# das-ankur/Efficient-PIC-with-Variance-Aware-Masking

Hardware: AMD Instinct MI355X
Metric: megapixels/sec encode+decode (g_a->mask->g_s) at 256x256 bs32 (higher is better)
Workload: dtype f32 (bf16x3 split operands); 1 GPU; forward_single_quality q=2.5 on 32x3x256x256 per GPU (dual g_a, hyperprior, 10 base + 10 progressive slices, variance mask, likelihood, LRP, g_s[1]); README model N=192 M=640; batch_per_gpu=32, global_batch=32, hip_graph=True, weights=synthetic seed 0

## Files before the change

efficient-pic-with-variance-aware-masking_amd/csrc/conv_igemm.hip:

```cpp
#include "common.h"
#include <cstdlib>

namespace vam {

typedef float f32x16 __attribute__((ext_vector_type(16)));
typedef unsigned int u32x4 __attribute__((ext_vector_type(4)));
typedef __bf16 bf16x8 __attribute__((ext_vector_type(8)));
typedef _Float16 f16x8 __attribute__((ext_vector_type(8)));
typedef _Float16 f16x2 __attribute__((ext_vector_type(2)));

struct ConvP {
  const float* seg_ptr[VAM_MAX_SEG];
  int seg_ld[VAM_MAX_SEG];
  int seg_end[VAM_MAX_SEG];
  int n_seg;
  int H, W, HW;
  int kh, kw, stride, pad_y, pad_x;
  int Ho, Wo, HoWo;
  int P;
  int N, Npad;
  int Cin, Kc, Kc16;
  const float* wpack;
  const float* bias;
  float* out;
  int ldo, Hf, Wf, osy, osx, ooy, oox, Cq, act, flags;
  const float* pre;
  const float* mul;
  const float* post;
  const float* post2;
  int ld_pre, ld_mul, ld_post, ld_post2;
  float* preact;
  int ld_preact;
  int tiles_n;
  const int* in_amax[VAM_MAX_SEG];
  int* out_amax;
};

constexpr int VAM_CONVI_DUAL = 1 << 29;
constexpr int VAM_CONVI_STAGED = 1 << 30;

struct GroupArgs {
  int nprob;
  int staged_epilogue;
  int tile_start[VAM_MAX_GROUP + 1];
  ConvP p[VAM_MAX_GROUP];
};

__device__ __forceinline__ float apply_act(float v, int act) {
  switch (act) {
    case VAM_ACT_GELU: return vam_gelu(v);
    case VAM_ACT_LEAKY: return v > 0.f ? v : v * 0.01f;
    case VAM_ACT_HALF_TANH: return 0.5f * tanhf(v);
    case VAM_ACT_SIGMOID: return 1.0f / (1.0f + expf(-v));
    case VAM_ACT_CLAMP01: return fminf(fmaxf(v, 0.f), 1.f);
    case VAM_ACT_RSQRT: return 1.0f / sqrtf(v);
    case VAM_ACT_SQRT: return sqrtf(v);
    case VAM_ACT_DOUBLE: return 2.0f * v;
    default: return v;
  }
}

constexpr int PK = 16;

template <int BM, int BN, int BK, int WGM, int WGN, int MODE, int AIN = 0, int SPEC = 0>
__global__ __launch_bounds__(WGM * WGN * 64 * (SPEC ? 2 : 1), SPEC ? ((BM + BN <= 192) ? 4 : 2) : (((MODE == 1 || MODE == 3) && BM == 128 && BN == 128) ? 3 : 2)) void conv_igemm_kernel(const GroupArgs args) {
  static_assert(SPEC == 0 || MODE == 1 || MODE == 3, "wave specialisation is built for the split-operand modes");
  static_assert(MODE != 3 || AIN == 0, "MODE 3 (fp16x2) takes fp32 inputs");
  static_assert(MODE != 2 || AIN <= 1, "MODE 2: AIN 0 = fp32 input rounded while staged, 1 = bf16 input");
  constexpr int NT = WGM * WGN * 64;
  constexpr int NTC = NT;
  constexpr int NTB = NT * (SPEC ? 2 : 1);
  constexpr int LDS_LD = BK;
  constexpr int TM = BM / WGM / 32;
  constexpr int TN = BN / WGN / 32;
  constexpr int CPR = MODE ? 4 : BK / 4;
  constexpr int LDW = MODE ? 8 : 4;
  static_assert(MODE == 0 || BK == 32, "the bf16 paths step K by 32 channels");
  constexpr int SW_SHIFT = (CPR == 4) ? 2 : 1;
  constexpr int RPP = NT / CPR;
  constexpr int NA = (BM + RPP - 1) / RPP;
  constexpr int NB = (BN + RPP - 1) / RPP;
  constexpr bool A_FULL = (BM % RPP) == 0, B_FULL = (BN % RPP) == 0;
  static_assert(TM >= 1 && TN >= 1 && BM == TM * WGM * 32 && BN == TN * WGN * 32, "tile/wave layout");

  extern __shared__ __attribute__((aligned(16))) float smem[];
  float* sA = smem;
  float* sB = smem + 2 * BM * LDS_LD;

  int pi = -1, t = 0;
  {
    const int xcd = blockIdx.x & 7;
    int idx = blockIdx.x >> 3;
#pragma unroll
    for (int i = 0; i < VAM_MAX_GROUP; ++i) {
      if (i < args.nprob && pi < 0) {
        const int T = args.tile_start[i + 1] - args.tile_start[i];
        const int q = T >> 3, r = T & 7;
        const int c = q + (xcd < r ? 1 : 0);
        if (idx < c) {
          pi = i;
          t = xcd * q + (xcd < r ? xcd : r) + idx;
        } else {
          idx -= c;
        }
      }
    }
  }
  if (pi < 0) return;
  const ConvP& P = args.p[pi];
  const int u_kh = __builtin_amdgcn_readfirstlane(P.kh), u_kw = __builtin_amdgcn_readfirstlane(P.kw);
  const int u_W = __builtin_amdgcn_readfirstlane(P.W), u_Kc = __builtin_amdgcn_readfirstlane(P.Kc);
  const int u_kc16 = __builtin_amdgcn_readfirstlane(P.Kc16), u_Npad = __builtin_amdgcn_readfirstlane(P.Npad);
  const int u_se0 = __builtin_amdgcn_readfirstlane(P.seg_end[0]), u_se1 = __builtin_amdgcn_readfirstlane(P.seg_end[1]);
  const int u_se2 = __builtin_amdgcn_readfirstlane(P.seg_end[2]);
  const int tn = t % P.tiles_n, tm = t / P.tiles_n;
  const int m0 = tm * BM, n0 = tn * BN;

  const bool is_loader = SPEC && (__builtin_amdgcn_readfirstlane((int)threadIdx.x >> 6) >= WGM * WGN);
  const int tid = (SPEC && (int)threadIdx.x >= NTC) ? (int)threadIdx.x - NTC : (int)threadIdx.x;
  const int lane = tid & 63, wid = tid >> 6;
  const int wm = wid / WGN, wn = wid % WGN;
  const int ld_row = tid / CPR;
  const int ld_col = (tid % CPR) * LDW;

  int a_pix0[NA];
  unsigned a_mask[NA];
#pragma unroll
  for (int i = 0; i < NA; ++i) {
    int p = m0 + ld_row + i * RPP;
    a_pix0[i] = 0;
    a_mask[i] = 0u;
    if (p < P.P && (A_FULL || ld_row + i * RPP < BM)) {
      int b = p / P.HoWo;
      int r = p - b * P.HoWo;
      int oy = r / P.Wo;
      int ox = r - oy * P.Wo;
      const int iy0 = oy * P.stride - P.pad_y, ix0 = ox * P.stride - P.pad_x;
      a_pix0[i] = b * P.HW + iy0 * P.W + ix0;
      unsigned m = 0u;
      for (int ty = 0; ty < u_kh; ++ty)
        for (int tx = 0; tx < u_kw; ++tx)
          if ((unsigned)(iy0 + ty) < (unsigned)P.H && (unsigned)(ix0 + tx) < (unsigned)P.W) m |= 1u << (ty * u_kw + tx);
      a_mask[i] = m;
    }
  }
  f32x16 acc[TM][TN];
  if constexpr (!SPEC) {
#pragma unroll
    for (int i = 0; i < TM; ++i)
#pragma unroll
      for (int j = 0; j < TN; ++j)
#pragma unroll
        for (int r = 0; r < 16; ++r) acc[i][j][r] = 0.f;
  }

  const int l31 = lane & 31, lh = lane >> 5;
  const unsigned long long wpa = reinterpret_cast<unsigned long long>(P.wpack);
  const __amdgpu_buffer_rsrc_t rsrc_w = __builtin_amdgcn_make_buffer_rsrc(
      reinterpret_cast<void*>(((unsigned long long)(unsigned)__builtin_amdgcn_readfirstlane((unsigned)(wpa >> 32)) << 32) |
                              (unsigned long long)(unsigned)__builtin_amdgcn_readfirstlane((unsigned)wpa)), 0, 0x7FFFFFFF, 0x00020000);
  const bool sq = (P.flags & VAM_CONV_SQUARE_IN) != 0;

  int c_ty = 0, c_tx = 0, c_kc = 0, c_tap = 0;
  int s_begin = 0, s_end = 0, s_ld4 = 0;
  unsigned s_lo = 0, s_hi = 0;
  const int n_taps = u_kh * u_kw;
  const bool dual = (MODE == 1 || MODE == 3) && (P.flags & VAM_CONVI_DUAL) != 0;
  const int n_chunks = dual ? (n_taps + 1) / 2 : n_taps * u_Kc;
  constexpr bool DIRECT_CFG = !SPEC && BM == 128 && BN == 64;
  const bool direct_out = DIRECT_CFG && !args.staged_epilogue &&
                          (P.flags & (VAM_CONV_OUT_NCHW | VAM_CONV_OUT_BF3 | VAM_CONV_OUT_BF16 | VAM_CONV_AUX_BF16 | VAM_CONVI_STAGED)) == 0;
  const int kc16 = u_kc16;
  if constexpr (MODE == 0) {
    unsigned b_off[NB];
  #pragma unroll
    for (int i = 0; i < NB; ++i) {
      const int r = ld_row + i * RPP;
      const bool ok = (B_FULL || r < BN) && (n0 + r < P.Npad);
      b_off[i] = ok ? (unsigned)((((ld_col >> 4) * u_Npad + n0 + r) * PK + (ld_col & 15)) * 4) : 0x80000000u;
    }
    float4 ra0[NA], rb0[NB], ra1[NA], rb1[NB];


    auto gload = [&](float4 (&ra)[NA], float4 (&rb)[NB]) {
      const int cc0 = c_kc * BK;
      if (cc0 < s_begin || cc0 >= s_end) {
        const int k = (cc0 >= u_se0 ? 1 : 0) + (cc0 >= u_se1 ? 1 : 0) + (cc0 >= u_se2 ? 1 : 0);
        s_begin = __builtin_amdgcn_readfirstlane(k ? P.seg_end[k - 1] : 0);
        s_end = __builtin_amdgcn_readfirstlane(P.seg_end[k]);
        const unsigned long long spa = reinterpret_cast<unsigned long long>(P.seg_ptr[k]);
        s_lo = (unsigned)__builtin_amdgcn_readfirstlane((unsigned)spa);
        s_hi = (unsigned)__builtin_amdgcn_readfirstlane((unsigned)(spa >> 32));
        s_ld4 = __builtin_amdgcn_readfirstlane(P.seg_ld[k]) * 4;
      }
      const int seg_begin = s_begin;
      const int sld4 = s_ld4;
      const __amdgpu_buffer_rsrc_t rsrc_a = __builtin_amdgcn_make_buffer_rsrc(
          reinterpret_cast<void*>(((unsigned long long)s_hi << 32) | s_lo), 0, 0x7FFFFFFF, 0x00020000);
      const int tap_pix = c_ty * u_W + c_tx;
      const int col4 = (cc0 - seg_begin + ld_col) * 4;
  #pragma unroll
      for (int i = 0; i < NA; ++i) {
        const bool ok = (a_mask[i] >> c_tap) & 1u;
        const unsigned off = (unsigned)((a_pix0[i] + tap_pix) * sld4 + col4);
        const u32x4 v = __builtin_amdgcn_raw_buffer_load_b128(rsrc_a, (int)(ok ? off : 0x80000000u), 0, 0);
        float4 f = make_float4(__uint_as_float(v.x), __uint_as_float(v.y), __uint_as_float(v.z), __uint_as_float(v.w));
        ra[i] = sq ? make_float4(f.x * f.x, f.y * f.y, f.z * f.z, f.w * f.w) : f;
      }
      const unsigned wbase = (unsigned)((c_tap * kc16 + c_kc * (BK / PK)) * u_Npad * (PK * 4));
  #pragma unroll
      for (int i = 0; i < NB; ++i) {
        const u32x4 v = __builtin_amdgcn_raw_buffer_load_b128(rsrc_w, (int)(b_off[i] + wbase), 0, 0);
        rb[i] = make_float4(__uint_as_float(v.x), __uint_as_float(v.y), __uint_as_float(v.z), __uint_as_float(v.w));
      }
      if (BK == 16) {
        const int has_half = (((c_kc & 1) == 0) && (c_kc + 1 < kc16)) ? 1 : 0;
        const int adv_tap = has_half ? 0 : 1;
        c_kc += has_half;
        c_tap += adv_tap;
        c_tx += adv_tap;
        const int wx = (c_tx == u_kw) ? 1 : 0;
        c_tx = wx ? 0 : c_tx;
        c_ty += wx;
        const int wt = (c_tap == n_taps) ? 1 : 0;
        c_tap = wt ? 0 : c_tap;
        c_ty = wt ? 0 : c_ty;
        c_kc = adv_tap ? (wt ? (c_kc | 1) + 1 : (c_kc & ~1)) : c_kc;
      } else {
        ++c_tap;
        ++c_tx;
        const int wx = (c_tx == u_kw) ? 1 : 0;
        c_tx = wx ? 0 : c_tx;
        c_ty += wx;
        const int wt = (c_tap == n_taps) ? 1 : 0;
        c_tap = wt ? 0 : c_tap;
        c_ty = wt ? 0 : c_ty;
        c_kc += wt;
      }
    };
    static_assert(RPP % 16 == 0, "the swizzle of a thread's rows must not depend on the pass");
    const int st_col = (((ld_col >> 2) ^ ((ld_row >> SW_SHIFT) & (CPR - 1))) << 2);
    auto sstore = [&](int buf, const float4 (&ra)[NA], const float4 (&rb)[NB]) {
      float* a = sA + buf * BM * LDS_LD;
      float* b = sB + buf * BN * LDS_LD;
  #pragma unroll
      for (int i = 0; i < NA; ++i)
        if (A_FULL || ld_row + i * RPP < BM)
          *reinterpret_cast<float4*>(a + (ld_row + i * RPP) * LDS_LD + st_col) = ra[i];
  #pragma unroll
      for (int i = 0; i < NB; ++i)
        if (B_FULL || ld_row + i * RPP < BN)
          *reinterpret_cast<float4*>(b + (ld_row + i * RPP) * LDS_LD + st_col) = rb[i];
    };

    const int a_row0 = (wm * TM * 32 + l31) * LDS_LD;
    const int b_row0 = (wn * TN * 32 + l31) * LDS_LD;
    const int rd_sw = (l31 >> SW_SHIFT) & (CPR - 1);
    int rd_col[BK / 8];
  #pragma unroll
    for (int kk = 0; kk < BK / 8; ++kk) rd_col[kk] = ((kk * 2 + lh) ^ rd_sw) << 2;

    auto compute = [&](int buf) {
      const float* a = sA + buf * BM * LDS_LD + a_row0;
      const float* b = sB + buf * BN * LDS_LD + b_row0;
      float4 fa[2][TM], fb[2][TN];
  #pragma unroll
      for (int i = 0; i < TM; ++i) fa[0][i] = *reinterpret_cast<const float4*>(a + i * 32 * LDS_LD + rd_col[0]);
  #pragma unroll
      for (int j = 0; j < TN; ++j) fb[0][j] = *reinterpret_cast<const float4*>(b + j * 32 * LDS_LD + rd_col[0]);
  #pragma unroll
      for (int kk = 0; kk < BK / 8; ++kk) {
        const int cur = kk & 1, nxt = cur ^ 1;
        if (kk + 1 < BK / 8) {
  #pragma unroll
          for (int i = 0; i < TM; ++i) fa[nxt][i] = *reinterpret_cast<const float4*>(a + i * 32 * LDS_LD + rd_col[kk + 1]);
  #pragma unroll
          for (int j = 0; j < TN; ++j) fb[nxt][j] = *reinterpret_cast<const float4*>(b + j * 32 * LDS_LD + rd_col[kk + 1]);
        }
  #pragma unroll
        for (int i = 0; i < TM; ++i)
  #pragma unroll
          for (int j = 0; j < TN; ++j) {
            acc[i][j] = __builtin_amdgcn_mfma_f32_32x32x2f32(fa[cur][i].x, fb[cur][j].x, acc[i][j], 0, 0, 0);
            acc[i][j] = __builtin_amdgcn_mfma_f32_32x32x2f32(fa[cur][i].y, fb[cur][j].y, acc[i][j], 0, 0, 0);
            acc[i][j] = __builtin_amdgcn_mfma_f32_32x32x2f32(fa[cur][i].z, fb[cur][j].z, acc[i][j], 0, 0, 0);
            acc[i][j] = __builtin_amdgcn_mfma_f32_32x32x2f32(fa[cur][i].w, fb[cur][j].w, acc[i][j], 0, 0, 0);
          }
      }
    };

    gload(ra0, rb0);
    sstore(0, ra0, rb0);
    if (n_chunks > 1) gload(ra0, rb0);
    __syncthreads();
    int ch = 0;
    for (; ch + 3 < n_chunks; ch += 2) {
      sstore(1, ra0, rb0);
      gload(ra1, rb1);
      compute(0);
      __syncthreads();
      sstore(0, ra1, rb1);
      gload(ra0, rb0);
      compute(1);
      __syncthreads();
    }
    for (; ch < n_chunks; ch += 2) {
      if (ch + 1 < n_chunks) sstore(1, ra0, rb0);
      if (ch + 2 < n_chunks) gload(ra1, rb1);
      compute(0);
      __syncthreads();
      if (ch + 1 >= n_chunks) break;
      if (ch + 2 < n_chunks) sstore(0, ra1, rb1);
      if (ch + 3 < n_chunks) gload(ra0, rb0);
      compute(1);
      __syncthreads();
    }

  } else if constexpr (MODE == 1 || MODE == 3) {
    constexpr bool F16 = MODE == 3;
    constexpr int NPL = F16 ? 2 : 3;
    constexpr int UPR = NPL * 4;
    constexpr int RS = NPL * 16;
    constexpr int NBUF = SPEC ? 2 : ((BM + BN <= 128) ? 2 : 1);
    constexpr int NBC = (BN * UPR + NT - 1) / NT;
    float* sA1 = smem;
    float* sB1 = smem + NBUF * BM * RS;
    unsigned b_goff[NBC];
    int b_loff[NBC];
#pragma unroll
    for (int j = 0; j < NBC; ++j) {
      const int idx = tid + j * NT;
      const int row = idx / UPR, c = idx - row * UPR;
      const bool in_tile = idx < BN * UPR;
      b_goff[j] = (in_tile && n0 + row < u_Npad) ? (unsigned)((n0 + row) * (UPR * 16) + c * 16) : 0x80000000u;
      b_loff[j] = in_tile ? row * RS + (F16 ? (c ^ ((row >> 1) & 7)) : ((c & ~3) | ((c & 3) ^ ((row >> 2) & 3)))) * 4 : -1;
    }
    const int u_Cin = __builtin_amdgcn_readfirstlane(P.Cin);
    float a_scale = 1.f, a_unscale = 1.f;
    if constexpr (F16) {
      int mb = 0;
#pragma unroll
      for (int k = 0; k < VAM_MAX_SEG; ++k)
        if (P.in_amax[k]) mb = max(mb, *P.in_amax[k]);
      float m = __uint_as_float((unsigned)__builtin_amdgcn_readfirstlane(mb));
      if (sq) m = m * m;
      const int e = (int)((__float_as_uint(m) >> 23) & 0xFFu) - 127;
      int sh = (m > 0.f && e > -127 && e < 128) ? 14 - e : 0;
      sh = sh > 126 ? 126 : (sh < -126 ? -126 : sh);
      a_scale = __uint_as_float((unsigned)(sh + 127) << 23);
      a_unscale = __uint_as_float((unsigned)(127 - sh) << 23);
    }
    constexpr int NAR = AIN ? 3 : 2;
    u32x4 ra0[NA][NAR], ra1[NA][NAR];
    u32x4 rb0[NBC], rb1[NBC];

    auto gload = [&](u32x4 (&ra)[NA][NAR], u32x4 (&rb)[NBC]) {
      const int cc0 = c_kc * 32;
      if (cc0 < s_begin || cc0 >= s_end) {
        const int k = (cc0 >= u_se0 ? 1 : 0) + (cc0 >= u_se1 ? 1 : 0) + (cc0 >= u_se2 ? 1 : 0);
        s_begin = __builtin_amdgcn_readfirstlane(k ? P.seg_end[k - 1] : 0);
        s_end = __builtin_amdgcn_readfirstlane(P.seg_end[k]);
        const unsigned long long spa = reinterpret_cast<unsigned long long>(P.seg_ptr[k]);
        s_lo = (unsigned)__builtin_amdgcn_readfirstlane((unsigned)spa);
        s_hi = (unsigned)__builtin_amdgcn_readfirstlane((unsigned)(spa >> 32));
        s_ld4 = __builtin_amdgcn_readfirstlane(P.seg_ld[k]) * (AIN ? 48 : 4);
      }
      const __amdgpu_buffer_rsrc_t rsrc_a = __builtin_amdgcn_make_buffer_rsrc(
          reinterpret_cast<void*>(((unsigned long long)s_hi << 32) | s_lo), 0, 0x7FFFFFFF, 0x00020000);
      int tap_pix = c_ty * u_W + c_tx;
      int col4 = AIN ? ((cc0 - s_begin + ld_col) >> 3) * 48 : (cc0 - s_begin + ld_col) * 4;
      bool ch_ok = cc0 + ld_col < u_Cin;
      int my_tap = c_tap;
      if (!AIN && dual) {
        const bool second = ld_col >= 16;
        const int txb = (c_tx + 1 == u_kw) ? 0 : c_tx + 1, tyb = (c_tx + 1 == u_kw) ? c_ty + 1 : c_ty;
        tap_pix = second ? tyb * u_W + txb : tap_pix;
        my_tap = second ? c_tap + 1 : c_tap;
        col4 = (ld_col & 15) * 4;
        ch_ok = my_tap < n_taps;
      }
#pragma unroll
      for (int i = 0; i < NA; ++i) {
        const bool ok = ch_ok && ((a_mask[i] >> my_tap) & 1u);
        const unsigned off = ok ? (unsigned)((a_pix0[i] + tap_pix) * s_ld4 + col4) : 0x80000000u;
#pragma unroll
        for (int q = 0; q < NAR; ++q) ra[i][q] = __builtin_amdgcn_raw_buffer_load_b128(rsrc_a, (int)(off + 16u * q), 0, 0);
      }
      const unsigned wbase = (unsigned)((dual ? (c_tap >> 1) : (c_tap * u_Kc + c_kc)) * u_Npad) * (unsigned)(UPR * 16);
#pragma unroll
      for (int j = 0; j < NBC; ++j) rb[j] = __builtin_amdgcn_raw_buffer_load_b128(rsrc_w, (int)(b_goff[j] + wbase), 0, 0);
      for (int step = 0; step < (dual ? 2 : 1); ++step) {
        ++c_tap;
        ++c_tx;
        const int wx = (c_tx == u_kw) ? 1 : 0;
        c_tx = wx ? 0 : c_tx;
        c_ty += wx;
      }
      const int wt = (c_tap >= n_taps) ? 1 : 0;
      c_tap = wt ? 0 : c_tap;
      c_ty = wt ? 0 : c_ty;
      c_tx = wt ? 0 : c_tx;
      c_kc += wt;
    };
    static_assert(RPP % 16 == 0, "the swizzle of a thread's rows must not depend on the pass");
    const int st1_col = (((ld_col >> 3) ^ ((ld_row >> 2) & 3)) << 2);
    const int st3_col[2] = {((((ld_col >> 3)) ^ ((ld_row >> 1) & 7)) << 2), (((4 + (ld_col >> 3)) ^ ((ld_row >> 1) & 7)) << 2)};
    auto sstore = [&](int buf, const u32x4 (&ra)[NA][NAR], const u32x4 (&rb)[NBC]) {
      float* a = sA1 + buf * BM * RS;
      float* b = sB1 + buf * BN * RS;
#pragma unroll
      for (int i = 0; i < NA; ++i)
        if (A_FULL || ld_row + i * RPP < BM) {
          if constexpr (AIN) {
            float* dst = a + (ld_row + i * RPP) * RS + st1_col;
            *reinterpret_cast<u32x4*>(dst) = ra[i][0];
            *reinterpret_cast<u32x4*>(dst + 16) = ra[i][1];
            *reinterpret_cast<u32x4*>(dst + 32) = ra[i][NAR - 1];
            continue;
          }
          float x[8] = {__uint_as_float(ra[i][0].x), __uint_as_float(ra[i][0].y), __uint_as_float(ra[i][0].z), __uint_as_float(ra[i][0].w),
                        __uint_as_float(ra[i][1].x), __uint_as_float(ra[i][1].y), __uint_as_float(ra[i][1].z), __uint_as_float(ra[i][1].w)};
          if (sq) {
#pragma unroll
            for (int e = 0; e < 8; ++e) x[e] = x[e] * x[e];
          }
          if constexpr (F16) {
            unsigned hw2[4], lw2[4];
#pragma unroll
            for (int q = 0; q < 4; ++q) {
              const float x0 = x[2 * q] * a_scale, x1 = x[2 * q + 1] * a_scale;
              const f16x2 h = {(_Float16)x0, (_Float16)x1};
              const f16x2 l = {(_Float16)(x0 - (float)h[0]), (_Float16)(x1 - (float)h[1])};
              hw2[q] = __builtin_bit_cast(unsigned, h);
              lw2[q] = __builtin_bit_cast(unsigned, l);
            }
            float* drow = a + (ld_row + i * RPP) * RS;
            u32x4 t;
            t.x = hw2[0]; t.y = hw2[1]; t.z = hw2[2]; t.w = hw2[3];
            *reinterpret_cast<u32x4*>(drow + st3_col[0]) = t;
            t.x = lw2[0]; t.y = lw2[1]; t.z = lw2[2]; t.w = lw2[3];
            *reinterpret_cast<u32x4*>(drow + st3_col[1]) = t;
            continue;
          }
          unsigned hb[8], mb[8], lb[8];
#pragma unroll
          for (int e = 0; e < 8; ++e) {
            hb[e] = __float_as_uint(x[e]);
            const float r1 = x[e] - __uint_as_float(hb[e] & 0xFFFF0000u);
            mb[e] = __float_as_uint(r1);
            lb[e] = __float_as_uint(r1 - __uint_as_float(mb[e] & 0xFFFF0000u));
          }
          unsigned hw[4], mw[4], lw[4];
#pragma unroll
          for (int q = 0; q < 4; ++q) {
            hw[q] = __builtin_amdgcn_perm(hb[2 * q + 1], hb[2 * q], 0x07060302u);
            mw[q] = __builtin_amdgcn_perm(mb[2 * q + 1], mb[2 * q], 0x07060302u);
            lw[q] = __builtin_amdgcn_perm(lb[2 * q + 1], lb[2 * q], 0x07060302u);
          }
          float* dst = a + (ld_row + i * RPP) * RS + st1_col;
          u32x4 t;
          t.x = hw[0]; t.y = hw[1]; t.z = hw[2]; t.w = hw[3];
          *reinterpret_cast<u32x4*>(dst) = t;
          t.x = mw[0]; t.y = mw[1]; t.z = mw[2]; t.w = mw[3];
          *reinterpret_cast<u32x4*>(dst + 16) = t;
          t.x = lw[0]; t.y = lw[1]; t.z = lw[2]; t.w = lw[3];
          *reinterpret_cast<u32x4*>(dst + 32) = t;
        }
#pragma unroll
      for (int j = 0; j < NBC; ++j) {
        if (b_loff[j] >= 0) *reinterpret_cast<u32x4*>(b + b_loff[j]) = rb[j];
      }
    };
    const int a_row1 = (wm * TM * 32 + l31) * RS;
    const int b_row1 = (wn * TN * 32 + l31) * RS;
    const int rsw = (l31 >> 2) & 3;
    const int rd1[2] = {((lh ^ rsw) << 2), (((2 + lh) ^ rsw) << 2)};
    const int rsw3 = (l31 >> 1) & 7;
    const int rd3[2][2] = {{((lh ^ rsw3) << 2), (((4 + lh) ^ rsw3) << 2)}, {(((2 + lh) ^ rsw3) << 2), (((6 + lh) ^ rsw3) << 2)}};
    auto compute = [&](int buf) {
      const float* a = sA1 + buf * BM * RS + a_row1;
      const float* b = sB1 + buf * BN * RS + b_row1;
      if constexpr (F16) {
#pragma unroll
        for (int ks = 0; ks < 2; ++ks) {
          f16x8 fa[TM][2], fb[TN][2];
#pragma unroll
          for (int i = 0; i < TM; ++i)
#pragma unroll
            for (int pl = 0; pl < 2; ++pl) fa[i][pl] = *reinterpret_cast<const f16x8*>(a + i * 32 * RS + rd3[ks][pl]);
#pragma unroll
          for (int j = 0; j < TN; ++j)
#pragma unroll
            for (int pl = 0; pl < 2; ++pl) fb[j][pl] = *reinterpret_cast<const f16x8*>(b + j * 32 * RS + rd3[ks][pl]);
#pragma unroll
          for (int i = 0; i < TM; ++i)
#pragma unroll
            for (int j = 0; j < TN; ++j) {
              acc[i][j] = __builtin_amdgcn_mfma_f32_32x32x16_f16(fa[i][0], fb[j][1], acc[i][j], 0, 0, 0);
              acc[i][j] = __builtin_amdgcn_mfma_f32_32x32x16_f16(fa[i][1], fb[j][0], acc[i][j], 0, 0, 0);
              acc[i][j] = __builtin_amdgcn_mfma_f32_32x32x16_f16(fa[i][0], fb[j][0], acc[i][j], 0, 0, 0);
            }
        }
        return;
      }
#pragma unroll
      for (int ks = 0; ks < 2; ++ks) {
        bf16x8 fa[TM][3], fb[TN][3];
#pragma unroll
        for (int i = 0; i < TM; ++i)
#pragma unroll
          for (int pl = 0; pl < 3; ++pl) fa[i][pl] = *reinterpret_cast<const bf16x8*>(a + i * 32 * RS + pl * 16 + rd1[ks]);
#pragma unroll
        for (int j = 0; j < TN; ++j)
#pragma unroll
          for (int pl = 0; pl < 3; ++pl) fb[j][pl] = *reinterpret_cast<const bf16x8*>(b + j * 32 * RS + pl * 16 + rd1[ks]);
#pragma unroll
        for (int i = 0; i < TM; ++i)
#pragma unroll
          for (int j = 0; j < TN; ++j) {
            acc[i][j] = __builtin_amdgcn_mfma_f32_32x32x16_bf16(fa[i][0], fb[j][2], acc[i][j], 0, 0, 0);
            acc[i][j] = __builtin_amdgcn_mfma_f32_32x32x16_bf16(fa[i][2], fb[j][0], acc[i][j], 0, 0, 0);
            acc[i][j] = __builtin_amdgcn_mfma_f32_32x32x16_bf16(fa[i][1], fb[j][1], acc[i][j], 0, 0, 0);
            acc[i][j] = __builtin_amdgcn_mfma_f32_32x32x16_bf16(fa[i][0], fb[j][1], acc[i][j], 0, 0, 0);
            acc[i][j] = __builtin_amdgcn_mfma_f32_32x32x16_bf16(fa[i][1], fb[j][0], acc[i][j], 0, 0, 0);
            acc[i][j] = __builtin_amdgcn_mfma_f32_32x32x16_bf16(fa[i][0], fb[j][0], acc[i][j], 0, 0, 0);
          }
        if constexpr (TN >= 7) __builtin_amdgcn_sched_barrier(0);
      }
    };
    auto unscale = [&]() {
      if constexpr (F16) {
        const float* wsc = P.wpack + (size_t)n_taps * u_Kc * u_Npad * 32;
#pragma unroll
        for (int j = 0; j < TN; ++j) {
          const int n = n0 + (wn * TN + j) * 32 + l31;
          const float f = (n < u_Npad ? wsc[n] : 0.f) * a_unscale;
#pragma unroll
          for (int i = 0; i < TM; ++i)
#pragma unroll
            for (int r = 0; r < 16; ++r) acc[i][j][r] *= f;
        }
      }
    };
    if constexpr (SPEC) {
      if (is_loader) {
        gload(ra0, rb0);
        if (n_chunks > 1) gload(ra1, rb1);
        sstore(0, ra0, rb0);
        if (n_chunks > 2) gload(ra0, rb0);
        __syncthreads();
        for (int ch = 0; ch < n_chunks; ch += 2) {
          if (ch + 1 < n_chunks) sstore(1, ra1, rb1);
          if (ch + 3 < n_chunks) gload(ra1, rb1);
          __syncthreads();
          if (ch + 1 >= n_chunks) break;
          if (ch + 2 < n_chunks) sstore(0, ra0, rb0);
          if (ch + 4 < n_chunks) gload(ra0, rb0);
          __syncthreads();
        }
      } else {
#pragma unroll
        for (int i = 0; i < TM; ++i)
#pragma unroll
          for (int j = 0; j < TN; ++j)
#pragma unroll
            for (int r = 0; r < 16; ++r) acc[i][j][r] = 0.f;
        __syncthreads();
        for (int ch = 0; ch < n_chunks; ch += 2) {
          compute(0);
          __syncthreads();
          if (ch + 1 >= n_chunks) break;
          compute(1);
          __syncthreads();
        }
        unscale();
        if (!direct_out) {
          float* sCf = smem;
#pragma unroll
          for (int i = 0; i < TM; ++i)
#pragma unroll
            for (int j = 0; j < TN; ++j)
#pragma unroll
              for (int r = 0; r < 16; ++r) {
                const int row = wm * TM * 32 + i * 32 + (r & 3) + 8 * (r >> 2) + 4 * lh;
                sCf[row * (BN + 4) + wn * TN * 32 + j * 32 + l31] = acc[i][j][r];
              }
        }
      }
    } else if constexpr (NBUF == 2) {
      gload(ra0, rb0);
      sstore(0, ra0, rb0);
      if (n_chunks > 1) gload(ra1, rb1);
      if (n_chunks > 2) gload(ra0, rb0);
      __syncthreads();
      int ch = 0;
      for (; ch + 1 < n_chunks; ch += 2) {
        sstore(1, ra1, rb1);
        if (ch + 3 < n_chunks) gload(ra1, rb1);
        compute(0);
        __syncthreads();
        if (ch + 2 < n_chunks) sstore(0, ra0, rb0);
        if (ch + 4 < n_chunks) gload(ra0, rb0);
        compute(1);
        __syncthreads();
      }
      if (ch < n_chunks) {
        compute(0);
        __syncthreads();
      }
      unscale();
    } else {
      gload(ra0, rb0);
      for (int ch = 0; ch < n_chunks; ++ch) {
        sstore(0, ra0, rb0);
        __syncthreads();
        if (ch + 1 < n_chunks) gload(ra0, rb0);
        compute(0);
        __syncthreads();
      }
      unscale();
    }
  } else {
    constexpr int RS = 16;
    constexpr int NBC = (BN * 4 + NT - 1) / NT;
    float* sA2 = smem;
    float* sB2 = smem + 2 * BM * RS;
    unsigned b_goff[NBC];
    int b_loff[NBC];
#pragma unroll
    for (int j = 0; j < NBC; ++j) {
      const int idx = tid + j * NT;
      const int row = idx >> 2, c = idx & 3;
      const bool in_tile = idx < BN * 4;
      b_goff[j] = (in_tile && n0 + row < u_Npad) ? (unsigned)((n0 + row) * 64 + c * 16) : 0x80000000u;
      b_loff[j] = in_tile ? row * RS + ((c ^ ((row >> 2) & 3)) << 2) : -1;
    }
    const int u_Cin = __builtin_amdgcn_readfirstlane(P.Cin);
    constexpr int NAR = AIN ? 1 : 2;
    u32x4 ra0[NA][NAR], ra1[NA][NAR];
    u32x4 rb0[NBC], rb1[NBC];
    auto gload = [&](u32x4 (&ra)[NA][NAR], u32x4 (&rb)[NBC]) {
      const int cc0 = c_kc * 32;
      if (cc0 < s_begin || cc0 >= s_end) {
        const int k = (cc0 >= u_se0 ? 1 : 0) + (cc0 >= u_se1 ? 1 : 0) + (cc0 >= u_se2 ? 1 : 0);
        s_begin = __builtin_amdgcn_readfirstlane(k ? P.seg_end[k - 1] : 0);
        s_end = __builtin_amdgcn_readfirstlane(P.seg_end[k]);
        const unsigned long long spa = reinterpret_cast<unsigned long long>(P.seg_ptr[k]);
        s_lo = (unsigned)__builtin_amdgcn_readfirstlane((unsigned)spa);
        s_hi = (unsigned)__builtin_amdgcn_readfirstlane((unsigned)(spa >> 32));
        s_ld4 = __builtin_amdgcn_readfirstlane(P.seg_ld[k]) * (AIN ? 2 : 4);
      }
      const __amdgpu_buffer_rsrc_t rsrc_a = __builtin_amdgcn_make_buffer_rsrc(
          reinterpret_cast<void*>(((unsigned long long)s_hi << 32) | s_lo), 0, 0x7FFFFFFF, 0x00020000);
      const int tap_pix = c_ty * u_W + c_tx;
      const int col4 = (cc0 - s_begin + ld_col) * (AIN ? 2 : 4);
      const bool ch_ok = cc0 + ld_col < u_Cin;
#pragma unroll
      for (int i = 0; i < NA; ++i) {
        const bool ok = ch_ok && ((a_mask[i] >> c_tap) & 1u);
        const unsigned off = ok ? (unsigned)((a_pix0[i] + tap_pix) * s_ld4 + col4) : 0x80000000u;
#pragma unroll
        for (int q = 0; q < NAR; ++q) ra[i][q] = __builtin_amdgcn_raw_buffer_load_b128(rsrc_a, (int)(off + 16u * q), 0, 0);
      }
      const unsigned wbase = (unsigned)((c_tap * u_Kc + c_kc) * u_Npad) * 64u;
#pragma unroll
      for (int j = 0; j < NBC; ++j) rb[j] = __builtin_amdgcn_raw_buffer_load_b128(rsrc_w, (int)(b_goff[j] + wbase), 0, 0);
      ++c_tap;
      ++c_tx;
      const int wx = (c_tx == u_kw) ? 1 : 0;
      c_tx = wx ? 0 : c_tx;
      c_ty += wx;
      const int wt = (c_tap == n_taps) ? 1 : 0;
      c_tap = wt ? 0 : c_tap;
      c_ty = wt ? 0 : c_ty;
      c_kc += wt;
    };
    auto pk2 = [](float lo, float hi) -> unsigned {
      const __bf16 a = (__bf16)lo, b = (__bf16)hi;
      return (unsigned)__builtin_bit_cast(unsigned short, a) | ((unsigned)__builtin_bit_cast(unsigned short, b) << 16);
    };
    const int st2_col = (((ld_col >> 3) ^ ((ld_row >> 2) & 3)) << 2);
    auto sstore = [&](int buf, const u32x4 (&ra)[NA][NAR], const u32x4 (&rb)[NBC]) {
      float* a = sA2 + buf * BM * RS;
      float* b = sB2 + buf * BN * RS;
#pragma unroll
      for (int i = 0; i < NA; ++i)
        if (A_FULL || ld_row + i * RPP < BM) {
          u32x4 t;
          if constexpr (AIN) {
            t = ra[i][0];
            if (sq) {
              unsigned w[4] = {t.x, t.y, t.z, t.w};
#pragma unroll
              for (int q = 0; q < 4; ++q) {
                const float lo = __uint_as_float(w[q] << 16), hi = __uint_as_float(w[q] & 0xFFFF0000u);
                w[q] = pk2(lo * lo, hi * hi);
              }
              t.x = w[0]; t.y = w[1]; t.z = w[2]; t.w = w[3];
            }
          } else {
            float x[8] = {__uint_as_float(ra[i][0].x), __uint_as_float(ra[i][0].y), __uint_as_float(ra[i][0].z), __uint_as_float(ra[i][0].w),
                          __uint_as_float(ra[i][NAR - 1].x), __uint_as_float(ra[i][NAR - 1].y), __uint_as_float(ra[i][NAR - 1].z), __uint_as_float(ra[i][NAR - 1].w)};
            if (sq) {
#pragma unroll
              for (int e = 0; e < 8; ++e) x[e] = x[e] * x[e];
            }
            t.x = pk2(x[0], x[1]); t.y = pk2(x[2], x[3]); t.z = pk2(x[4], x[5]); t.w = pk2(x[6], x[7]);
          }
          *reinterpret_cast<u32x4*>(a + (ld_row + i * RPP) * RS + st2_col) = t;
        }
#pragma unroll
      for (int j = 0; j < NBC; ++j)
        if (b_loff[j] >= 0) *reinterpret_cast<u32x4*>(b + b_loff[j]) = rb[j];
    };
    const int a_row2 = (wm * TM * 32 + l31) * RS;
    const int b_row2 = (wn * TN * 32 + l31) * RS;
    const int rsw = (l31 >> 2) & 3;
    const int rd2[2] = {((lh ^ rsw) << 2), (((2 + lh) ^ rsw) << 2)};
    auto compute = [&](int buf) {
      const float* a = sA2 + buf * BM * RS + a_row2;
      const float* b = sB2 + buf * BN * RS + b_row2;
#pragma unroll
      for (int ks = 0; ks < 2; ++ks) {
        bf16x8 fa[TM], fb[TN];
#pragma unroll
        for (int i = 0; i < TM; ++i) fa[i] = *reinterpret_cast<const bf16x8*>(a + i * 32 * RS + rd2[ks]);
#pragma unroll
        for (int j = 0; j < TN; ++j) fb[j] = *reinterpret_cast<const bf16x8*>(b + j * 32 * RS + rd2[ks]);
#pragma unroll
        for (int i = 0; i < TM; ++i)
#pragma unroll
          for (int j = 0; j < TN; ++j) acc[i][j] = __builtin_amdgcn_mfma_f32_32x32x16_bf16(fa[i], fb[j], acc[i][j], 0, 0, 0);
      }
    };
    gload(ra0, rb0);
    sstore(0, ra0, rb0);
    if (n_chunks > 1) gload(ra1, rb1);
    if (n_chunks > 2) gload(ra0, rb0);
    __syncthreads();
    int ch = 0;
    for (; ch + 1 < n_chunks; ch += 2) {
      sstore(1, ra1, rb1);
      if (ch + 3 < n_chunks) gload(ra1, rb1);
      compute(0);
      __syncthreads();
      if (ch + 2 < n_chunks) sstore(0, ra0, rb0);
      if (ch + 4 < n_chunks) gload(ra0, rb0);
      compute(1);
      __syncthreads();
    }
    if (ch < n_chunks) {
      compute(0);
      __syncthreads();
    }
  }

  constexpr int LDC = BN + 4;
  constexpr int SROWS = SPEC ? BM : WGM * 32;
  float* sC = smem;
  int* sPix = reinterpret_cast<int*>(smem + SROWS * LDC);
  const bool ps2 = (P.flags & VAM_CONV_PS2) != 0;
  const bool nchw = (P.flags & VAM_CONV_OUT_NCHW) != 0;
  const bool dense = !ps2 && !nchw && P.osy == 1 && P.osx == 1 && P.ooy == 0 && P.oox == 0 &&
                     P.Hf == P.Ho && P.Wf == P.Wo;
  const bool vec_ok = !nchw && (!ps2 || (P.Cq & 3) == 0);
  const bool out_p3 = (P.flags & VAM_CONV_OUT_BF3) != 0;
  const bool out16 = (P.flags & VAM_CONV_OUT_BF16) != 0;
  const bool aux16 = (P.flags & VAM_CONV_AUX_BF16) != 0;
#ifdef VAM_NO_TRAIN_EPILOGUE
  const bool mulg = false;
#define VAM_PREACT(P) false
#else
  const bool mulg = (P.flags & VAM_CONV_MUL_GELU_GRAD) != 0;
#define VAM_PREACT(P) ((P).preact != nullptr)
#endif
  auto ld_aux = [&](const float* base, size_t off) -> float4 {
    if (aux16) {
      const uint2 u = *reinterpret_cast<const uint2*>(reinterpret_cast<const unsigned short*>(base) + off);
      return make_float4(__uint_as_float(u.x << 16), __uint_as_float(u.x & 0xFFFF0000u), __uint_as_float(u.y << 16),
                         __uint_as_float(u.y & 0xFFFF0000u));
    }
    return *reinterpret_cast<const float4*>(base + off);
  };
  const int Cc = ps2 ? P.Cq : P.N;
  const size_t HfWf = (size_t)P.Hf * P.Wf;
  auto decode_row = [&](int row, int slot) {
    const int p = m0 + row;
    int pix = p, ob = 0;
    if (!dense && p < P.P) {
      ob = p / P.HoWo;
      int rr = p - ob * P.HoWo;
      int oy = rr / P.Wo;
      int ox = rr - oy * P.Wo;
      if (ps2) pix = (ob * P.Hf + 2 * oy) * P.Wf + 2 * ox;
      else pix = (ob * P.Hf + oy * P.osy + P.ooy) * P.Wf + ox * P.osx + P.oox;
    }
    sPix[2 * slot] = pix;
    sPix[2 * slot + 1] = ob;
  };
  float omax = 0.f;
  const bool pub = P.out_amax != nullptr;
  auto publish = [&]() {
    if (pub) {
      float m = omax;
#pragma unroll
      for (int o = 32; o; o >>= 1) m = fmaxf(m, __shfl_xor(m, o));
      if ((threadIdx.x & 63) == 0 && m > 0.f && __float_as_int(m) > __hip_atomic_load(P.out_amax, __ATOMIC_RELAXED, __HIP_MEMORY_SCOPE_AGENT))
        atomicMax(P.out_amax, __float_as_int(m));
    }
  };
  auto emit = [&](int srow, int row, int c4) {
    const int p = m0 + row;
    const int n = n0 + c4;
    if (p >= P.P || n >= P.N) return;
    const float4 av = *reinterpret_cast<const float4*>(sC + srow * LDC + c4);
    float v[4] = {av.x, av.y, av.z, av.w};
    const int pixb = sPix[2 * srow], ob = sPix[2 * srow + 1];
    if (vec_ok) {
      int cch = n;
      size_t opix = (size_t)pixb;
      if (ps2) {
        int ph = n / P.Cq;
        cch = n - ph * P.Cq;
        opix += (size_t)(ph >> 1) * P.Wf + (ph & 1);
      }
      if (P.bias) {
        const float4 bb = *reinterpret_cast<const float4*>(P.bias + n);
        v[0] += bb.x; v[1] += bb.y; v[2] += bb.z; v[3] += bb.w;
      }
      if (P.pre) {
        const float4 t4 = ld_aux(P.pre, opix * P.ld_pre + cch);
        v[0] += t4.x; v[1] += t4.y; v[2] += t4.z; v[3] += t4.w;
      }
      if (VAM_PREACT(P)) *reinterpret_cast<float4*>(P.preact + opix * P.ld_preact + cch) = make_float4(v[0], v[1], v[2], v[3]);
#pragma unroll
      for (int k = 0; k < 4; ++k) v[k] = apply_act(v[k], P.act);
      if (P.mul) {
        float4 t4 = ld_aux(P.mul, opix * P.ld_mul + cch);
        if (mulg) t4 = make_float4(vam_gelu_grad(t4.x), vam_gelu_grad(t4.y), vam_gelu_grad(t4.z), vam_gelu_grad(t4.w));
        v[0] *= t4.x; v[1] *= t4.y; v[2] *= t4.z; v[3] *= t4.w;
      }
      if (P.post) {
        const float4 t4 = ld_aux(P.post, opix * P.ld_post + cch);
        v[0] += t4.x; v[1] += t4.y; v[2] += t4.z; v[3] += t4.w;
      }
      if (P.post2) {
        const float4 t4 = ld_aux(P.post2, opix * P.ld_post2 + cch);
        v[0] += t4.x; v[1] += t4.y; v[2] += t4.z; v[3] += t4.w;
      }
      if (pub) omax = fmaxf(omax, fmaxf(fmaxf(fabsf(v[0]), fabsf(v[1])), fmaxf(fabsf(v[2]), fabsf(v[3]))));
      if (out_p3) {
        unsigned hb[4], mb[4], lb[4];
#pragma unroll
        for (int k = 0; k < 4; ++k) {
          hb[k] = __float_as_uint(v[k]);
          const float r1 = v[k] - __uint_as_float(hb[k] & 0xFFFF0000u);
          mb[k] = __float_as_uint(r1);
          lb[k] = __float_as_uint(r1 - __uint_as_float(mb[k] & 0xFFFF0000u));
        }
        char* o3 = reinterpret_cast<char*>(P.out) + (opix * P.ldo + (size_t)(cch >> 3)) * 48 + (cch & 7) * 2;
        *reinterpret_cast<uint2*>(o3) = make_uint2(__builtin_amdgcn_perm(hb[1], hb[0], 0x07060302u), __builtin_amdgcn_perm(hb[3], hb[2], 0x07060302u));
        *reinterpret_cast<uint2*>(o3 + 16) = make_uint2(__builtin_amdgcn_perm(mb[1], mb[0], 0x07060302u), __builtin_amdgcn_perm(mb[3], mb[2], 0x07060302u));
        *reinterpret_cast<uint2*>(o3 + 32) = make_uint2(__builtin_amdgcn_perm(lb[1], lb[0], 0x07060302u), __builtin_amdgcn_perm(lb[3], lb[2], 0x07060302u));
      } else if (out16) {
        const __bf16 h0 = (__bf16)v[0], h1 = (__bf16)v[1], h2 = (__bf16)v[2], h3 = (__bf16)v[3];
        *reinterpret_cast<uint2*>(reinterpret_cast<unsigned short*>(P.out) + opix * P.ldo + cch) =
            make_uint2((unsigned)__builtin_bit_cast(unsigned short, h0) | ((unsigned)__builtin_bit_cast(unsigned short, h1) << 16),
                       (unsigned)__builtin_bit_cast(unsigned short, h2) | ((unsigned)__builtin_bit_cast(unsigned short, h3) << 16));
      } else {
        *reinterpret_cast<float4*>(P.out + opix * P.ldo + cch) = make_float4(v[0], v[1], v[2], v[3]);
      }
    } else {
      for (int k = 0; k < 4; ++k) {
        const int nn = n + k;
        if (nn >= P.N) break;
        int cch = nn;
        size_t opix = (size_t)pixb;
        if (ps2) {
          int ph = nn / P.Cq;
          cch = nn - ph * P.Cq;
          opix += (size_t)(ph >> 1) * P.Wf + (ph & 1);
        }
        float x = v[k] + (P.bias ? P.bias[nn] : 0.f);
        if (P.pre) x = x + P.pre[opix * P.ld_pre + cch];
        if (VAM_PREACT(P)) P.preact[opix * P.ld_preact + cch] = x;
        x = apply_act(x, P.act);
        if (P.mul) x = x * (mulg ? vam_gelu_grad(P.mul[opix * P.ld_mul + cch]) : P.mul[opix * P.ld_mul + cch]);
        if (P.post) x = x + P.post[opix * P.ld_post + cch];
        if (P.post2) x = x + P.post2[opix * P.ld_post2 + cch];
// ... 837 lines not shown
```

Measured before the change: 77.67 MP/s.

## Remap 128x224 wave-specialised tile to 2x2 block ownership per consumer wave

For the SPEC kernel with a 128x224 tile and 4x1 consumer waves, each wave pair now shares two 32-row A blocks. Each wave takes a side-dependent subset of 32-column B blocks: three blocks per A row plus a shared last column. Each wave therefore loads 2 A fragments and 4 B fragments per k-step instead of 1 A and 7 B, which cuts LDS read traffic and fragment registers. The epilogue and unscale index computations are remapped to match. The sched_barrier for wide TN is dropped, and the odd/even wave split adds template duplication and code size.

```diff
diff --git a/efficient-pic-with-variance-aware-masking_amd/csrc/conv_igemm.hip b/efficient-pic-with-variance-aware-masking_amd/csrc/conv_igemm.hip
--- a/efficient-pic-with-variance-aware-masking_amd/csrc/conv_igemm.hip
+++ b/efficient-pic-with-variance-aware-masking_amd/csrc/conv_igemm.hip
@@ -1,5 +1,6 @@
 #include "common.h"
 #include <cstdlib>
+#include <type_traits>
 
 namespace vam {
 
@@ -82,6 +83,14 @@
   constexpr int NB = (BN + RPP - 1) / RPP;
   constexpr bool A_FULL = (BM % RPP) == 0, B_FULL = (BN % RPP) == 0;
   static_assert(TM >= 1 && TN >= 1 && BM == TM * WGM * 32 && BN == TN * WGN * 32, "tile/wave layout");
+  constexpr bool MAP22 = SPEC && BM == 128 && BN == 224;
+  static_assert(!MAP22 || (WGM == 4 && WGN == 1), "the 2x2 block map is laid out for 4x1 consumer waves");
+  constexpr int NFA = MAP22 ? 2 : TM, NFB = MAP22 ? 4 : TN;
+  auto blk_a = [](int i, int j, int S) constexpr { return MAP22 ? (j < 6 ? j / 3 : S) : i; };
+  auto blk_b = [](int j) constexpr { return MAP22 ? (j < 6 ? j % 3 : 3) : j; };
+  auto frag_col = [](int f, int S) constexpr { return MAP22 ? (f < 3 ? 4 * S + f : 3) : f; };
+  constexpr std::integral_constant<int, 0> side0{};
+  constexpr std::integral_constant<int, 1> side1{};
 
   extern __shared__ __attribute__((aligned(16))) float smem[];
   float* sA = smem;
@@ -120,6 +129,9 @@
   const int tid = (SPEC && (int)threadIdx.x >= NTC) ? (int)threadIdx.x - NTC : (int)threadIdx.x;
   const int lane = tid & 63, wid = tid >> 6;
   const int wm = wid / WGN, wn = wid % WGN;
+  const int u_wid = __builtin_amdgcn_readfirstlane(wid);
+  const int w_rb = MAP22 ? (u_wid & ~1) : wm * TM;
+  const int w_cb = wn * TN;
   const int ld_row = tid / CPR;
   const int ld_col = (tid % CPR) * LDW;
 
@@ -471,69 +483,73 @@
         if (b_loff[j] >= 0) *reinterpret_cast<u32x4*>(b + b_loff[j]) = rb[j];
       }
     };
-    const int a_row1 = (wm * TM * 32 + l31) * RS;
-    const int b_row1 = (wn * TN * 32 + l31) * RS;
+    const int a_row1 = (w_rb * 32 + l31) * RS;
+    const int b_row1 = (w_cb * 32 + l31) * RS;
     const int rsw = (l31 >> 2) & 3;
     const int rd1[2] = {((lh ^ rsw) << 2), (((2 + lh) ^ rsw) << 2)};
     const int rsw3 = (l31 >> 1) & 7;
     const int rd3[2][2] = {{((lh ^ rsw3) << 2), (((4 + lh) ^ rsw3) << 2)}, {(((2 + lh) ^ rsw3) << 2), (((6 + lh) ^ rsw3) << 2)}};
-    auto compute = [&](int buf) {
+    auto compute_s = [&](int buf, auto side) {
+      constexpr int S = decltype(side)::value;
       const float* a = sA1 + buf * BM * RS + a_row1;
       const float* b = sB1 + buf * BN * RS + b_row1;
       if constexpr (F16) {
 #pragma unroll
         for (int ks = 0; ks < 2; ++ks) {
-          f16x8 fa[TM][2], fb[TN][2];
+          f16x8 fa[NFA][2], fb[NFB][2];
+#pragma unroll
+          for (int i = 0; i < NFA; ++i)
+#pragma unroll
+            for (int pl = 0; pl < 2; ++pl) fa[i][pl] = *reinterpret_cast<const f16x8*>(a + i * 32 * RS + rd3[ks][pl]);
+#pragma unroll
+          for (int j = 0; j < NFB; ++j)
+#pragma unroll
+            for (int pl = 0; pl < 2; ++pl) fb[j][pl] = *reinterpret_cast<const f16x8*>(b + frag_col(j, S) * 32 * RS + rd3[ks][pl]);
 #pragma unroll
           for (int i = 0; i < TM; ++i)
 #pragma unroll
-            for (int pl = 0; pl < 2; ++pl) fa[i][pl] = *reinterpret_cast<const f16x8*>(a + i * 32 * RS + rd3[ks][pl]);
-#pragma unroll
-          for (int j = 0; j < TN; ++j)
-#pragma unroll
-            for (int pl = 0; pl < 2; ++pl) fb[j][pl] = *reinterpret_cast<const f16x8*>(b + j * 32 * RS + rd3[ks][pl]);
-#pragma unroll
-          for (int i = 0; i < TM; ++i)
-#pragma unroll
             for (int j = 0; j < TN; ++j) {
-              acc[i][j] = __builtin_amdgcn_mfma_f32_32x32x16_f16(fa[i][0], fb[j][1], acc[i][j], 0, 0, 0);
-              acc[i][j] = __builtin_amdgcn_mfma_f32_32x32x16_f16(fa[i][1], fb[j][0], acc[i][j], 0, 0, 0);
-              acc[i][j] = __builtin_amdgcn_mfma_f32_32x32x16_f16(fa[i][0], fb[j][0], acc[i][j], 0, 0, 0);
+              const int ai = blk_a(i, j, S), bj = blk_b(j);
+              acc[i][j] = __builtin_amdgcn_mfma_f32_32x32x16_f16(fa[ai][0], fb[bj][1], acc[i][j], 0, 0, 0);
+              acc[i][j] = __builtin_amdgcn_mfma_f32_32x32x16_f16(fa[ai][1], fb[bj][0], acc[i][j], 0, 0, 0);
+              acc[i][j] = __builtin_amdgcn_mfma_f32_32x32x16_f16(fa[ai][0], fb[bj][0], acc[i][j], 0, 0, 0);
             }
         }
         return;
       }
 #pragma unroll
       for (int ks = 0; ks < 2; ++ks) {
-        bf16x8 fa[TM][3], fb[TN][3];
+        bf16x8 fa[NFA][3], fb[NFB][3];
+#pragma unroll
+        for (int i = 0; i < NFA; ++i)
+#pragma unroll
+          for (int pl = 0; pl < 3; ++pl) fa[i][pl] = *reinterpret_cast<const bf16x8*>(a + i * 32 * RS + pl * 16 + rd1[ks]);
+#pragma unroll
+        for (int j = 0; j < NFB; ++j)
+#pragma unroll
+          for (int pl = 0; pl < 3; ++pl) fb[j][pl] = *reinterpret_cast<const bf16x8*>(b + frag_col(j, S) * 32 * RS + pl * 16 + rd1[ks]);
 #pragma unroll
         for (int i = 0; i < TM; ++i)
 #pragma unroll
-          for (int pl = 0; pl < 3; ++pl) fa[i][pl] = *reinterpret_cast<const bf16x8*>(a + i * 32 * RS + pl * 16 + rd1[ks]);
-#pragma unroll
-        for (int j = 0; j < TN; ++j)
-#pragma unroll
-          for (int pl = 0; pl < 3; ++pl) fb[j][pl] = *reinterpret_cast<const bf16x8*>(b + j * 32 * RS + pl * 16 + rd1[ks]);
-#pragma unroll
-        for (int i = 0; i < TM; ++i)
-#pragma unroll
           for (int j = 0; j < TN; ++j) {
-            acc[i][j] = __builtin_amdgcn_mfma_f32_32x32x16_bf16(fa[i][0], fb[j][2], acc[i][j], 0, 0, 0);
-            acc[i][j] = __builtin_amdgcn_mfma_f32_32x32x16_bf16(fa[i][2], fb[j][0], acc[i][j], 0, 0, 0);
-            acc[i][j] = __builtin_amdgcn_mfma_f32_32x32x16_bf16(fa[i][1], fb[j][1], acc[i][j], 0, 0, 0);
-            acc[i][j] = __builtin_amdgcn_mfma_f32_32x32x16_bf16(fa[i][0], fb[j][1], acc[i][j], 0, 0, 0);
-            acc[i][j] = __builtin_amdgcn_mfma_f32_32x32x16_bf16(fa[i][1], fb[j][0], acc[i][j], 0, 0, 0);
-            acc[i][j] = __builtin_amdgcn_mfma_f32_32x32x16_bf16(fa[i][0], fb[j][0], acc[i][j], 0, 0, 0);
+            const int ai = blk_a(i, j, S), bj = blk_b(j);
+            acc[i][j] = __builtin_amdgcn_mfma_f32_32x32x16_bf16(fa[ai][0], fb[bj][2], acc[i][j], 0, 0, 0);
+            acc[i][j] = __builtin_amdgcn_mfma_f32_32x32x16_bf16(fa[ai][2], fb[bj][0], acc[i][j], 0, 0, 0);
+            acc[i][j] = __builtin_amdgcn_mfma_f32_32x32x16_bf16(fa[ai][1], fb[bj][1], acc[i][j], 0, 0, 0);
+            acc[i][j] = __builtin_amdgcn_mfma_f32_32x32x16_bf16(fa[ai][0], fb[bj][1], acc[i][j], 0, 0, 0);
+            acc[i][j] = __builtin_amdgcn_mfma_f32_32x32x16_bf16(fa[ai][1], fb[bj][0], acc[i][j], 0, 0, 0);
+            acc[i][j] = __builtin_amdgcn_mfma_f32_32x32x16_bf16(fa[ai][0], fb[bj][0], acc[i][j], 0, 0, 0);
           }
-        if constexpr (TN >= 7) __builtin_amdgcn_sched_barrier(0);
       }
     };
-    auto unscale = [&]() {
+    auto compute = [&](int buf) { compute_s(buf, side0); };
+    auto unscale_s = [&](auto side) {
       if constexpr (F16) {
+        constexpr int S = decltype(side)::value;
         const float* wsc = P.wpack + (size_t)n_taps * u_Kc * u_Npad * 32;
 #pragma unroll
         for (int j = 0; j < TN; ++j) {
-          const int n = n0 + (wn * TN + j) * 32 + l31;
+          const int n = n0 + (w_cb + frag_col(blk_b(j), S)) * 32 + l31;
           const float f = (n < u_Npad ? wsc[n] : 0.f) * a_unscale;
 #pragma unroll
           for (int i = 0; i < TM; ++i)
@@ -542,6 +558,7 @@
         }
       }
     };
+    auto unscale = [&]() { unscale_s(side0); };
     if constexpr (SPEC) {
       if (is_loader) {
         gload(ra0, rb0);
@@ -566,25 +583,48 @@
 #pragma unroll
             for (int r = 0; r < 16; ++r) acc[i][j][r] = 0.f;
         __syncthreads();
-        for (int ch = 0; ch < n_chunks; ch += 2) {
-          compute(0);
-          __syncthreads();
-          if (ch + 1 >= n_chunks) break;
-          compute(1);
-          __syncthreads();
-        }
-        unscale();
-        if (!direct_out) {
-          float* sCf = smem;
-#pragma unroll
-          for (int i = 0; i < TM; ++i)
-#pragma unroll
-            for (int j = 0; j < TN; ++j)
-#pragma unroll
-              for (int r = 0; r < 16; ++r) {
-                const int row = wm * TM * 32 + i * 32 + (r & 3) + 8 * (r >> 2) + 4 * lh;
-                sCf[row * (BN + 4) + wn * TN * 32 + j * 32 + l31] = acc[i][j][r];
-              }
+        auto consume = [&](auto side) {
+          constexpr int S = decltype(side)::value;
+          if constexpr (MAP22) {
+            int ch = 0;
+            for (; ch + 1 < n_chunks; ch += 2) {
+              compute_s(0, side);
+              __syncthreads();
+              compute_s(1, side);
+              __syncthreads();
+            }
+            if (ch < n_chunks) {
+              compute_s(0, side);
+              __syncthreads();
+            }
+          } else {
+            for (int ch = 0; ch < n_chunks; ch += 2) {
+              compute_s(0, side);
+              __syncthreads();
+              if (ch + 1 >= n_chunks) break;
+              compute_s(1, side);
+              __syncthreads();
+            }
+          }
+          unscale_s(side);
+          if (!direct_out) {
+            float* sCf = smem;
+#pragma unroll
+            for (int i = 0; i < TM; ++i)
+#pragma unroll
+              for (int j = 0; j < TN; ++j)
+#pragma unroll
+                for (int r = 0; r < 16; ++r) {
+                  const int row = (w_rb + blk_a(i, j, S)) * 32 + (r & 3) + 8 * (r >> 2) + 4 * lh;
+                  sCf[row * (BN + 4) + (w_cb + frag_col(blk_b(j), S)) * 32 + l31] = acc[i][j][r];
+                }
+          }
+        };
+        if constexpr (MAP22) {
+          if (u_wid & 1) consume(side1);
+          else consume(side0);
+        } else {
+          consume(side0);
         }
       }
     } else if constexpr (NBUF == 2) {
```

New measurement: 78.99 MP/s (median of 6 runs). 1.02x the previous value.
